# luciddreamer-cvlab/LucidDreamer

Measured on AMD Instinct MI355X. Metric: views/sec fwd+bwd @1080p (1e6 Gaussians), higher is better.
Workload: dtype f32

## Files before the change

luciddreamer_amd/csrc/api.hip:

```cpp
#include "common.h"
#include "lr_src_hash.h"

#include <cstdio>
#include <cstdlib>
#include <cstddef>
#include <cstring>
#include <cmath>
#include <initializer_list>
#include <map>
#include <atomic>
#include <chrono>
#include <mutex>
#include <thread>
#include <string>
#include <vector>

namespace {

thread_local std::string g_last_error;

int fail(int code, const std::string& msg)
{
    g_last_error = msg;
    return code;
}

bool weight_ok(float w) { return w >= 0.f && std::isfinite(w); }

#define LR_HIP_CHECK(expr)                                                                        \
    do {                                                                                          \
        hipError_t e__ = (expr);                                                                  \
        if (e__ != hipSuccess)                                                                    \
            return fail(LR_ERR_HIP, std::string(#expr) + ": " + hipGetErrorString(e__));          \
    } while (0)

#define LR_DEBUG_SYNC(debug, stream, what)                                                        \
    do {                                                                                          \
        if (debug) {                                                                              \
            hipError_t e__ = hipStreamSynchronize(stream);                                        \
            if (e__ == hipSuccess) e__ = hipGetLastError();                                       \
            if (e__ != hipSuccess)                                                                \
                return fail(LR_ERR_HIP, std::string("[HIP ERROR] after ") + what + ": " + hipGetErrorString(e__)); \
        }                                                                                         \
    } while (0)

enum Stage { ST_PREPROCESS = 0, ST_COMPACT, ST_BIN_COUNT, ST_BIN_SCAN, ST_BIN_SCATTER, ST_TILE_SORT, ST_RENDER_FWD,
             ST_GRAD_ZERO, ST_RENDER_BWD, ST_OUT_ZERO, ST_GAUSS_BWD, ST_COUNT };
const char* const kStageNames[ST_COUNT] = { "preprocess", "compact", "bin_count", "bin_scan", "bin_scatter", "tile_sort",
                                            "render_fwd", "grad_zero", "render_bwd", "out_zero", "gauss_bwd" };
struct ProfRec { int stage; hipEvent_t e0, e1; };
bool g_prof_on = false;
std::mutex g_prof_mu;
std::vector<ProfRec> g_prof_recs;
std::vector<hipEvent_t> g_prof_pool;

hipEvent_t prof_event()
{
    {
        std::lock_guard<std::mutex> lock(g_prof_mu);
        if (!g_prof_pool.empty()) { hipEvent_t e = g_prof_pool.back(); g_prof_pool.pop_back(); return e; }
    }
    hipEvent_t e = nullptr;
    (void)hipEventCreate(&e);
    return e;
}
struct ProfScope {
    hipStream_t s; ProfRec r; bool on;
    ProfScope(int stage, hipStream_t s_) : s(s_), on(g_prof_on)
    {
        if (on) { r.stage = stage; r.e0 = prof_event(); r.e1 = prof_event(); (void)hipEventRecord(r.e0, s); }
    }
    ~ProfScope()
    {
        if (on) { (void)hipEventRecord(r.e1, s); std::lock_guard<std::mutex> lock(g_prof_mu); g_prof_recs.push_back(r); }
    }
};

struct BinProf : lr::TileBinTimes {
    ProfRec cur; bool open = false;
    void mark(int boundary, hipStream_t s) override
    {
        if (!g_prof_on) return;
        if (open) { (void)hipEventRecord(cur.e1, s); std::lock_guard<std::mutex> lock(g_prof_mu); g_prof_recs.push_back(cur); open = false; }
        if (boundary < 4) {
            cur.stage = ST_BIN_COUNT + boundary; cur.e0 = prof_event(); cur.e1 = prof_event();
            (void)hipEventRecord(cur.e0, s); open = true;
        }
    }
};

struct TuneTable { int v[lr::TUNE_COUNT]; TuneTable() { for (int& x : v) x = -1; } } g_tune_table;
int* const g_tune = g_tune_table.v;
const char* const kTuneNames[] = { "bwd_red", "blend_quad", "tile_map", "preprocess", "gauss_bwd", "tsort", "walk_own", "hit_mask", "views_in_flight", "strict", "part_scan", "bwd_seg", "fwd_pair", "pcull" };
static_assert(sizeof(kTuneNames) / sizeof(kTuneNames[0]) == lr::TUNE_COUNT, "one name per TuneKey");

std::mutex g_hint_mu;
std::map<std::pair<int, uint32_t>, float> g_vis_frac;
std::map<std::pair<int, uint32_t>, uint32_t> g_inst_hint;
constexpr float kSparseViewFraction = 0.30f;

void view_hint_note(int device, uint32_t P, uint32_t num_compact, uint32_t num_instances)
{
    if (P == 0) return;
    std::lock_guard<std::mutex> lock(g_hint_mu);
    g_vis_frac[std::make_pair(device, P)] = (float)num_compact / (float)P;
    g_inst_hint[std::make_pair(device, P)] = num_instances;
}
long long view_hint_instances(int device, uint32_t P)
{
    std::lock_guard<std::mutex> lock(g_hint_mu);
    auto it = g_inst_hint.find(std::make_pair(device, P));
    return it != g_inst_hint.end() ? (long long)it->second : -1;
}
bool view_hint_sparse(int device, uint32_t P)
{
    std::lock_guard<std::mutex> lock(g_hint_mu);
    auto it = g_vis_frac.find(std::make_pair(device, P));
    return it != g_vis_frac.end() && it->second <= kSparseViewFraction;
}

thread_local bool g_early_request = false;
thread_local long long g_early_ticket = -1;

struct StreamScratch { uint32_t* words = nullptr; size_t n = 0; bool dirty = false; };
std::mutex g_scratch_mu;
std::map<std::pair<int, hipStream_t>, StreamScratch> g_scratch;
StreamScratch* stream_scratch(hipStream_t s, size_t n_words)
{
    int device = 0;
    if (hipGetDevice(&device) != hipSuccess) return nullptr;
    StreamScratch* sc;
    {
        std::lock_guard<std::mutex> lock(g_scratch_mu);
        sc = &g_scratch[std::make_pair(device, s)];
    }
    if (sc->n < n_words) {
        uint32_t* w = nullptr;
        const size_t cap = n_words + n_words / 2 + 64;
        if (hipMalloc(reinterpret_cast<void**>(&w), cap * 4) != hipSuccess) return nullptr;
        if (hipMemsetAsync(w, 0, cap * 4, s) != hipSuccess) return nullptr;
        sc->words = w; sc->n = cap; sc->dirty = false;
    } else if (sc->dirty) {
        if (hipMemsetAsync(sc->words, 0, sc->n * 4, s) != hipSuccess) return nullptr;
        sc->dirty = false;
    }
    return sc;
}

constexpr int kLogSlots = 4096, kLogWords = 12;
constexpr long long kLogTicketBit = 1ll << 40;
struct ForwardLog { uint32_t* host = nullptr; uint32_t* dev = nullptr; std::atomic<long long> next{0}; };
std::mutex g_log_mu;
std::map<int, ForwardLog*> g_logs;
ForwardLog* forward_log(int device)
{
    std::lock_guard<std::mutex> lock(g_log_mu);
    auto it = g_logs.find(device);
    if (it != g_logs.end()) return it->second;
    ForwardLog* L = new ForwardLog();
    const size_t bytes = (size_t)kLogSlots * kLogWords * 4;
    if (hipHostMalloc(reinterpret_cast<void**>(&L->host), bytes, hipHostMallocMapped | hipHostMallocCoherent) != hipSuccess ||
        hipHostGetDevicePointer(reinterpret_cast<void**>(&L->dev), L->host, 0) != hipSuccess) {
        delete L;
        g_logs[device] = nullptr;
        return nullptr;
    }
    std::memset(L->host, 0, bytes);
    g_logs[device] = L;
    return L;
}
thread_local long long g_last_forward_ticket = -1;

thread_local hipEvent_t g_bwd_wait_event = nullptr;
hipEvent_t take_backward_wait_event() { hipEvent_t e = g_bwd_wait_event; g_bwd_wait_event = nullptr; return e; }

thread_local bool g_reset_sticky = false;
// ... 186 lines not shown
    if (P > 0 && (!v.means3D || !v.opacities || !radii)) return fail(LR_ERR_INVALID_ARG, "means3D/opacities/radii are required");
    if (P > 0 && v.shs == nullptr && v.colors_precomp == nullptr)
        return fail(LR_ERR_INVALID_ARG, "For non-RGB, provide precomputed Gaussian colors!");
    if (P > 0 && v.cov3D_precomp == nullptr && (v.scales == nullptr || v.rotations == nullptr))
        return fail(LR_ERR_INVALID_ARG, "provide scales+rotations or cov3D_precomp");
    if (v.shs != nullptr && (D < 0 || D > 3 || (D + 1) * (D + 1) > M))
        return fail(LR_ERR_INVALID_ARG, "SH degree must be 0..3 and (D+1)^2 <= M");
    if (binning_capacity < 0 || binning_capacity > 0xFFFFFFF0ll) return fail(LR_ERR_INVALID_ARG, "bad binning_capacity");

    const ViewParams vp = view_params(v);
    const int num_tiles = vp.gx * vp.gy;

    char* geom = a.geom_alloc(geom_layout(P).total, a.geom_user);
    char* img = a.img_alloc(img_layout(width, height).total, a.img_user);
    if (!geom || !img) return fail(LR_ERR_ALLOC, "geom/img allocator returned NULL");
    const GeomView gv = geom_view(geom, P);
    const ImgView iv = img_view(img, width, height);
    BinView bv = {};

    const size_t n_sum_words = chunk_sum_words(P);
    StreamScratch* scratch = P > 0 ? stream_scratch(s, n_sum_words) : nullptr;
    if (P > 0 && !scratch) return fail(LR_ERR_ALLOC, "could not allocate the per-stream scratch");
    struct DirtyOnError { StreamScratch* sc; bool armed; ~DirtyOnError() { if (sc && armed) sc->dirty = true; } } guard{ scratch, false };
    g_last_forward_ticket = -1;

    long long R_bound = 0;
    int num_rendered = 0;
    bool ranges_written = false;
    long long inst_hint = -1;

    if (P > 0) {
        int device = 0;
        (void)hipGetDevice(&device);
        inst_hint = view_hint_instances(device, (uint32_t)P);
        { ProfScope ps(ST_PREPROCESS, s);
        launch_preprocess(vp, v, a.prefiltered != 0, radii, gv, scratch->words, view_hint_sparse(device, (uint32_t)P), antialiasing, s); }
        guard.armed = true;
        LR_DEBUG_SYNC(debug, s, "preprocess");

        uint32_t* log_slot = nullptr;
        uint32_t log_tag = 0;
#ifdef LR_DIAGNOSTICS
        static const bool no_log = [] { const char* e = getenv("LR_NO_FWD_LOG"); return e && atoi(e) != 0; }();
#else
        constexpr bool no_log = false;
#endif
        if (binning_capacity != 0 && !no_log) {
            if (ForwardLog* L = forward_log(device)) {
                const long long seq = L->next.fetch_add(1);
                log_slot = L->dev + (size_t)(seq % kLogSlots) * kLogWords;
                log_tag = (uint32_t)(seq + 1);
                g_last_forward_ticket = ((long long)device << 41) | kLogTicketBit | (seq & (kLogTicketBit - 1));
            }
        }
        { ProfScope ps(ST_COMPACT, s);
        launch_compact(P, gv, reinterpret_cast<const uint4*>(scratch->words), (uint32_t)binning_capacity, log_slot, log_tag,
                       { iv.bin_total, (uint32_t)part_plan(num_tiles).bins }, reset_sticky, s); }
        LR_DEBUG_SYNC(debug, s, "compact");

        if (binning_capacity == 0) {
            GeomHeader h;
            LR_HIP_CHECK(hipMemcpyAsync(&h, gv.header, offsetof(GeomHeader, n_seg), hipMemcpyDeviceToHost, s));
            LR_HIP_CHECK(hipStreamSynchronize(s));
            view_hint_note(device, (uint32_t)P, h.num_compact, h.num_instances);
            R_bound = h.num_instances;
            if (h.num_rendered > 0x7FFFFFFFu)
                return fail(LR_ERR_INVALID_ARG, "num_rendered exceeds INT_MAX: use async mode (binning_capacity > 0) and read the count with lr_check");
            num_rendered = (int)h.num_rendered;
        } else {
            R_bound = binning_capacity;
            num_rendered = LR_NUM_RENDERED_ON_DEVICE;
            if (early_header) {
                g_early_ticket = g_last_forward_ticket >= 0 ? g_last_forward_ticket : lr_header_post(geom, a.stream);
                if (g_early_ticket < 0) return (int)g_early_ticket;
            }
        }

        char* bin = a.binning_alloc(bin_layout(R_bound).total, a.binning_user);
        if (!bin) return fail(LR_ERR_ALLOC, "binning allocator returned NULL");
        bv = bin_view(bin, R_bound);
        if (R_bound > 0) {
            BinProf bp;
            const int rc = launch_tile_binning(vp, bits_for((uint32_t)(R_bound - 1)), gv, iv, bv, radii, R_bound, &bp,
                                               { scratch->words, (uint32_t)n_sum_words }, s);
            if (rc == -2) return fail(LR_ERR_INVALID_ARG, "image / instance count too large: tile and slot bits exceed the 64-bit sort word");
            if (rc != 0) return fail(LR_ERR_HIP, "could not reserve LDS for the binning kernels");
            ranges_written = true;
            guard.armed = false;
            LR_DEBUG_SYNC(debug, s, "tile binning");
        }
    } else {
        (void)a.binning_alloc(bin_layout(0).total, a.binning_user);
    }
    if (!ranges_written) LR_HIP_CHECK(hipMemsetAsync(iv.ranges, 0, (size_t)num_tiles * sizeof(uint2), s));

    { ProfScope ps(ST_RENDER_FWD, s);
    launch_render_fwd(vp, gv, iv, bv, v.background, a.out_color, a.out_depth, inst_hint, s); }
    LR_DEBUG_SYNC(debug, s, "render");
    LR_HIP_CHECK(hipGetLastError());

    if (binning_capacity == 0 && a.prefiltered && P > 0) {
        uint32_t trap = 0;
        LR_HIP_CHECK(hipMemcpyAsync(&trap, &gv.header->prefilter_trap, 4, hipMemcpyDeviceToHost, s));
        LR_HIP_CHECK(hipStreamSynchronize(s));
        if (trap) return fail(LR_ERR_PREFILTERED, "Point is filtered although prefiltered is set. This shouldn't happen!");
    }
    return num_rendered;
}

static const char* const kUncoveredMsg =
    "lr_backward: R / binning_capacity are smaller than the forward's -- the blend backward's launch did not reach every list "
    "segment and the gradients of this view are incomplete (pass the value lr_forward returned / was given)";

static void zero_fill_write_rows(const lr::GradOut& out, float* dL_dsh_rest, int P, int M, bool raw, hipStream_t s)
{
    using namespace lr;
    const unsigned int accumulate_mask = out.accumulate_mask;
    float* const dL_dmean2D_abs = out.mean2D_abs;
    const unsigned long long Pn = (unsigned long long)P;
    const unsigned long long nsh = raw ? 3 * Pn : (unsigned long long)M * 3 * Pn;
    const unsigned long long nf[ACC_ROWS] = { 3 * Pn, 4 * Pn, Pn, 3 * Pn, 3 * Pn, 6 * Pn, nsh, 3 * Pn, 4 * Pn };
    float* zp[11]; unsigned long long zn[11]; int zc = 0;
    const bool no_fill = (accumulate_mask & LR_ACC_NO_ZERO_FILL) != 0u;
    for (int k = 0; k < ACC_ROWS; k++)
        if (out.row[k] != nullptr && !((accumulate_mask >> k) & 1u) && (!no_fill || k == ACC_MEAN2D)) { zp[zc] = out.row[k]; zn[zc] = nf[k]; zc++; }
    if (!no_fill && raw && dL_dsh_rest != nullptr && M > 1 && !((accumulate_mask >> ACC_SH) & 1u) && zc < 9) {
        zp[zc] = dL_dsh_rest; zn[zc] = (unsigned long long)(M - 1) * 3 * Pn; zc++;
    }
    const bool abs_own = dL_dmean2D_abs != nullptr && zc >= 9;
    if (dL_dmean2D_abs != nullptr && !abs_own) { zp[zc] = dL_dmean2D_abs; zn[zc] = 3 * Pn; zc++; }
    if (zc > 0) {
        ProfScope ps(ST_OUT_ZERO, s);
        launch_zero_outputs(zp, zn, zc, s);
        if (abs_own) { float* one = dL_dmean2D_abs; const unsigned long long n = 3 * Pn; launch_zero_outputs(&one, &n, 1, s); }
    }
}

static int backward_core(const lr_backward_args& a, hipEvent_t wait_before_accumulate, float* acc16, float* stat_accum = nullptr,
                         bool stat_abs = false)
{
    using namespace lr;
    const bool antialiasing = g_antialiasing.load(std::memory_order_relaxed) != 0;
    const lr_view& v = a.view;
    const int P = v.P, M = v.M, width = v.width, height = v.height, debug = a.debug;
    const bool raw = v.raw != 0;
    char* const geom_buffer = a.geom_buffer; char* const binning_buffer = a.binning_buffer; char* const image_buffer = a.image_buffer;
    const unsigned int accumulate_mask = a.accumulate_mask;
    const bool depth = a.dL_depths != nullptr && a.depth_image != nullptr;
    hipStream_t s = reinterpret_cast<hipStream_t>(a.stream);
    if (P <= 0) return 0;
    if (!geom_buffer || !binning_buffer || !image_buffer) return fail(LR_ERR_INVALID_ARG, "scratch buffers are required");
    if (!a.dL_dpix || !a.dL_dmean2D || !a.dL_dopacity || !a.dL_dmean3D)
        return fail(LR_ERR_INVALID_ARG, "gradient outputs dL_dmean2D/dL_dopacity/dL_dmean3D are required");
    if (v.colors_precomp != nullptr && !a.dL_dcolor) return fail(LR_ERR_INVALID_ARG, "dL_dcolor is required with colors_precomp");
    if (v.cov3D_precomp != nullptr && !a.dL_dcov3D) return fail(LR_ERR_INVALID_ARG, "dL_dcov3D is required with cov3D_precomp");
    if (v.scales != nullptr && (!a.dL_dscale || !a.dL_drot)) return fail(LR_ERR_INVALID_ARG, "dL_dscale/dL_drot are required with scales");
    if (v.shs != nullptr && a.dL_dsh == nullptr) return fail(LR_ERR_INVALID_ARG, "dL_dsh is required when shs is given");
    if (const int rc = all_aligned16("backward", "gradient outputs", { a.dL_dmean2D, a.dL_dconic, a.dL_dopacity, a.dL_dcolor, a.dL_dmean3D,
                                     a.dL_dcov3D, a.dL_dsh, a.dL_dscale, a.dL_drot, a.dL_dsh_rest, a.dL_dmean2D_abs })) return rc;

    const GeomView gv = geom_view(geom_buffer, P);
    const ImgView iv = img_view(image_buffer, width, height);
    const BinView bv = bin_view_list(binning_buffer);
    const long long seg_bound = (a.binning_capacity > 0 || a.R > 0)
                                    ? bin_seg_capacity(a.binning_capacity > 0 ? a.binning_capacity : (long long)a.R) : -1;

    const ViewParams vp = view_params(v, true, a.dL_dsh_rest);
// ... 1594 lines not shown
int lr_step_abort(void)
{
    int device = 0;
    LR_HIP_CHECK(hipGetDevice(&device));
    std::lock_guard<std::mutex> lock(g_step_mu);
    StepAcc& g = g_step[device];
    g.active = false; g.armed = false;
    return 0;
}

long long lr_forward_ticket(void) { return g_last_forward_ticket; }
void lr_backward_wait_event(void* event) { g_bwd_wait_event = reinterpret_cast<hipEvent_t>(event); }

static int forward_log_poll(long long ticket, int block, unsigned int* out8)
{
    const int device = (int)(ticket >> 41);
    const long long seq = ticket & (kLogTicketBit - 1);
    ForwardLog* L;
    {
        std::lock_guard<std::mutex> lock(g_log_mu);
        auto it = g_logs.find(device);
        L = it == g_logs.end() ? nullptr : it->second;
    }
    if (!L) return fail(LR_ERR_INVALID_ARG, "lr_header_poll: unknown forward-log ticket");
    const uint32_t want = (uint32_t)(seq + 1);
    volatile uint32_t* slot = L->host + (size_t)(seq % kLogSlots) * kLogWords;
    const auto t0 = std::chrono::steady_clock::now();
    for (int spin = 0;; spin++) {
        const uint32_t tag = __atomic_load_n(const_cast<uint32_t*>(slot), __ATOMIC_ACQUIRE);
        if (tag == want) break;
        if (tag != 0 && (int32_t)(tag - want) > 0)
            return fail(LR_ERR_INVALID_ARG, "lr_header_poll: the forward log has wrapped past this ticket (more than 4096 forwards were outstanding)");
        if (!block) return 0;
        if ((spin & 63) == 63) {
            std::this_thread::yield();
            if (std::chrono::steady_clock::now() - t0 > std::chrono::seconds(30))
                return fail(LR_ERR_HIP, "lr_header_poll: the forward of this ticket did not reach its scan within 30 s");
        }
    }
    if (out8) for (int i = 0; i < 8; i++) out8[i] = slot[1 + i];
    view_hint_note(device, slot[1 + LR_HDR_WORD(P)], slot[1 + LR_HDR_WORD(num_compact)], slot[1 + LR_HDR_WORD(num_instances)]);
    return 1;
}

int lr_header_poll(long long ticket, int block, unsigned int* out8)
{
    if (ticket >= 0 && (ticket & kLogTicketBit)) return forward_log_poll(ticket, block, out8);
    HeaderTicket h;
    {
        std::lock_guard<std::mutex> lock(g_hdr_mu);
        if (ticket < 0 || (size_t)ticket >= g_hdr_tickets.size() || !g_hdr_tickets[(size_t)ticket].busy)
            return fail(LR_ERR_INVALID_ARG, "lr_header_poll: unknown ticket");
        h = g_hdr_tickets[(size_t)ticket];
    }
    hipError_t q = block ? hipEventSynchronize(h.ev) : hipEventQuery(h.ev);
    if (q == hipErrorNotReady) return 0;
    if (q != hipSuccess) {
        header_ticket_release(ticket);
        return fail(LR_ERR_HIP, std::string("lr_header_poll: ") + hipGetErrorString(q));
    }
    if (out8) for (int i = 0; i < 8; i++) out8[i] = h.host[i];
    view_hint_note(h.device, h.host[LR_HDR_WORD(P)], h.host[LR_HDR_WORD(num_compact)], h.host[LR_HDR_WORD(num_instances)]);
    header_ticket_release(ticket);
    return 1;
}

void lr_request_early_header(void) { g_early_request = true; g_early_ticket = -1; }
long long lr_take_early_ticket(void) { const long long t = g_early_ticket; g_early_ticket = -1; g_early_request = false; return t; }

int lr_set_antialiasing(int on) { return g_antialiasing.exchange(on != 0 ? 1 : 0); }
int lr_get_antialiasing(void) { return g_antialiasing.load(); }

int lr_tune_set(const char* name, int value)
{
    if (!name) return fail(LR_ERR_INVALID_ARG, "lr_tune_set: NULL name");
    for (int i = 0; i < lr::TUNE_COUNT; i++)
        if (std::strcmp(name, kTuneNames[i]) == 0) {
#ifndef LR_DIAGNOSTICS
            if ((i == lr::TUNE_PART_SCAN && value >= 0) || (i == lr::TUNE_BWD_RED && (value == 0 || value == 2 || value == 3)) ||
                (i == lr::TUNE_FWD_PAIR && value == 1))
                return fail(LR_ERR_INVALID_ARG, std::string("lr_tune_set: ") + name + " = " + std::to_string(value) +
                            " selects a retired kernel (diagnostics build only: python -m luciddreamer_amd.build --diagnostics)");
#endif
            g_tune[i] = value;
            return 0;
        }
    return fail(LR_ERR_INVALID_ARG, std::string("lr_tune_set: unknown knob ") + name);
}

int lr_last_launch_shapes(int* forward_shape, int* backward_shape)
{
    if (forward_shape) *forward_shape = lr::last_fwd_shape();
    if (backward_shape) *backward_shape = lr::last_bwd_shape();
    return 0;
}

int lr_last_forward_channels(int* channels)
{
    if (channels) *channels = lr::last_fwd_channels();
    return 0;
}

int lr_profile_enable(int on)
{
    std::lock_guard<std::mutex> lock(g_prof_mu);
    for (auto& r : g_prof_recs) { g_prof_pool.push_back(r.e0); g_prof_pool.push_back(r.e1); }
    g_prof_recs.clear();
    g_prof_on = on != 0;
    return ST_COUNT;
}

const char* lr_profile_stage_name(int stage) { return (stage >= 0 && stage < ST_COUNT) ? kStageNames[stage] : ""; }

int lr_profile_read(double* ms_per_stage, long long* calls_per_stage, int n_stages)
{
    if (!ms_per_stage || !calls_per_stage || n_stages < ST_COUNT) return fail(LR_ERR_INVALID_ARG, "need ST_COUNT slots");
    for (int i = 0; i < n_stages; i++) { ms_per_stage[i] = 0.0; calls_per_stage[i] = 0; }
    std::lock_guard<std::mutex> lock(g_prof_mu);
    for (auto& r : g_prof_recs) {
        LR_HIP_CHECK(hipEventSynchronize(r.e1));
        float ms = 0.f;
        LR_HIP_CHECK(hipEventElapsedTime(&ms, r.e0, r.e1));
        ms_per_stage[r.stage] += ms;
        calls_per_stage[r.stage] += 1;
    }
    return ST_COUNT;
}

size_t lr_dist2_workspace_bytes(int P) { return lr::dist2_workspace_bytes(P); }

int lr_dist2_workspace_layout(int P, size_t offsets[4])
{
    if (P < 0) return fail(LR_ERR_INVALID_ARG, "P must be >= 0");
    if (!offsets) return fail(LR_ERR_INVALID_ARG, "NULL argument");
    lr::dist2_workspace_layout(P, offsets);
    return 0;
}

int lr_dist2(int P, const float* points, float* out, char* workspace, void* stream_)
{
    hipStream_t s = reinterpret_cast<hipStream_t>(stream_);
    if (P < 0) return fail(LR_ERR_INVALID_ARG, "P must be >= 0");
    if (P == 0) return 0;
    if (!points || !out || !workspace) return fail(LR_ERR_INVALID_ARG, "NULL argument");
    lr::launch_dist2(P, points, out, workspace, s);
    LR_HIP_CHECK(hipGetLastError());
    return 0;
}

}
```

luciddreamer_amd/csrc/common.h:

```cpp
#pragma once
#include <hip/hip_runtime.h>
#include <stdint.h>
#include <stddef.h>
#include "screen_cull.h"
#include "gauss_project.h"
#include "../../include/lucid_raster.h"

namespace lr {

constexpr int TILE_PIX = TILE_X * TILE_Y;
constexpr int WAVE = 64;

struct __attribute__((aligned(16))) GaussRec {
    float x, y, ca, cb;
    float cc, opacity, r, g;
    float b, depth, qmax, pad1;
};
static_assert(sizeof(GaussRec) == 48, "GaussRec must be 48 bytes");

struct __attribute__((aligned(16))) GradRec {
    float dmx, dmy, dca, dcb;
    float dcc, dop, dr, dg;
    float db, pad0, pad1, pad2;
};
// ... 201 lines not shown
{
#pragma clang fp contract(off)
    const float t = Cp * dy;
    return t * dy;
}
__device__ __forceinline__ float gauss_power1(float Ap, float Bd, float Cdd, float dx)
{
    return __builtin_fmaf(__builtin_fmaf(Ap, dx, Bd), dx, Cdd);
}
template <bool STRICT>
__device__ __forceinline__ void gauss_row(float qB, float qC, float dy, float& r0, float& r1)
{
    if (STRICT) { r0 = dy; r1 = 0.f; }
    else { r0 = gauss_bd(qB, dy); r1 = gauss_cdd(qC, dy); }
}
__device__ __forceinline__ float gauss_power_strict(float ca, float cb, float cc, float dx, float dy)
{
#pragma clang fp contract(off)
    return -0.5f * (ca * dx * dx + cc * dy * dy) - cb * dx * dy;
}
__device__ __forceinline__ float strict_expf(float x)
{
#pragma clang fp contract(off)
    const float c = 0x1.715476p+0f, cc = 0x1.4ae0bep-26f;
    const float ph = x * c;
    const float pl = __builtin_fmaf(x, cc, __builtin_fmaf(x, c, -ph));
    const float e = __builtin_rintf(ph);
    const float a = (ph - e) + pl;
    return __builtin_ldexpf(__builtin_amdgcn_exp2f(a), (int)e);
}
template <bool STRICT>
__device__ __forceinline__ float gauss_weight(float qA, float qB, float qC, float r0, float r1, float dx, float& power)
{
    if (STRICT) {
        power = gauss_power_strict(qA, qB, qC, dx, r0);
        return strict_expf(power);
    }
    power = gauss_power1(qA, r0, r1, dx);
    return __builtin_amdgcn_exp2f(power);
}

constexpr float LOG2E = 1.4426950408889634f;
constexpr float LN2 = 0.6931471805599453f;
__device__ __forceinline__ float gauss_exp2(float power2) { return __builtin_amdgcn_exp2f(power2); }

struct ViewParams {
    const float* view;
    const float* proj;
    const float* campos;
    float tan_fovx, tan_fovy, focal_x, focal_y, scale_modifier;
    int W, H, gx, gy, P, D, M;
    int hit_origin_limit;
    int raw;
    const float* sh_rest;
    const float* opacity_raw;
    float* dL_dsh_rest;
    ScreenCull cull;
    int pcull;
};

__device__ __forceinline__ float act_scale(float s) { return expf(s); }
__device__ __forceinline__ float act_opacity(float o) { return 1.0f / (1.0f + expf(-o)); }
__device__ __forceinline__ float act_quat_inv_norm(float r, float x, float y, float z)
{
    return 1.0f / fmaxf(sqrtf(r * r + x * x + y * y + z * z), 1e-12f);
}

struct WordSpan { uint32_t* words; uint32_t n; };
void launch_preprocess(const ViewParams& vp, const lr_view& v, bool prefiltered, int* radii, const GeomView& g,
                       uint32_t* chunk_sums, bool sparse_view_hint, bool antialiasing, hipStream_t s);
inline size_t chunk_sum_words(int P) { return 4 * (((size_t)(P > 0 ? P : 1) + SCAN_TILE - 1) / SCAN_TILE) + 1; }
void launch_mark_visible(int P, const float* means3D, const float* view, const float* proj, uint8_t* present,
                         hipStream_t s);

inline int radix_sort_passes(int end_bit) { return (end_bit + RADIX_BITS - 1) / RADIX_BITS; }
void radix_sort_pairs(uint32_t* key_a, uint32_t* key_b, uint32_t* val_a, uint32_t* val_b, bool vals_iota,
                      const uint32_t* n_dev, long long n_bound, int end_bit, uint32_t* hist,
                      uint32_t** keys_out, uint32_t** vals_out, hipStream_t s);

void launch_compact(int P, const GeomView& g, const uint4* block_sums, uint32_t capacity, uint32_t* log_slot, uint32_t log_tag,
                    WordSpan zero, bool reset_sticky, hipStream_t s);
struct TileBinTimes { virtual void mark(int boundary, hipStream_t s) = 0; virtual ~TileBinTimes() {} };
int launch_tile_binning(const ViewParams& vp, int slot_bits, const GeomView& g, const ImgView& im, const BinView& b,
                        const int* radii, long long bin_bound_hint, TileBinTimes* t, WordSpan clear, hipStream_t s);

enum TuneKey { TUNE_BWD_RED = 0, TUNE_BLEND_QUAD, TUNE_TILE_MAP, TUNE_PREPROCESS, TUNE_GAUSS_BWD, TUNE_TSORT, TUNE_WALK_OWN, TUNE_HIT_MASK, TUNE_VIEWS_IN_FLIGHT, TUNE_STRICT, TUNE_PART_SCAN, TUNE_BWD_SEG, TUNE_FWD_PAIR, TUNE_PCULL, TUNE_COUNT };
int tune_get(int key);

enum { BLEND_HALF = 0, BLEND_QUAD = 1, BLEND_TILE = 2 };
int blend_shape(int num_tiles, long long inst_bound = -1);
struct ViewsInFlight { explicit ViewsInFlight(int n); ~ViewsInFlight(); int prev; };
int views_in_flight();
void note_fwd_shape(int shape);
int last_fwd_shape();
int last_bwd_shape();
enum { FWD_CHANNEL_COLOR = 1, FWD_CHANNEL_DEPTH = 2 };
void note_fwd_channels(int channels);
int last_fwd_channels();
enum { TILE_MAP_BANDS = 0, TILE_MAP_PLAIN = 1 };
int blend_tile_map(int num_tiles);
__device__ __forceinline__ int blend_tile(int map, int num_tiles)
{
    int t = (int)blockIdx.x;
    if (map == TILE_MAP_BANDS) {
        const int per = (num_tiles + 7) >> 3;
        t = (int)(blockIdx.x & 7) * per + (int)(blockIdx.x >> 3);
    }
    return t < num_tiles ? t : -1;
}
void launch_render_fwd(const ViewParams& vp, const GeomView& g, const ImgView& im, const BinView& b, const float* bg,
                       float* out_color, float* out_depth, long long inst_hint, hipStream_t s);
void launch_render_alpha(const float* final_T, long long n, float* alpha, hipStream_t s);
void launch_render_median(int W, int H, int P, const GeomView& g, const ImgView& im, const char* bin_base, float* out_depth,
                          int* out_ids, hipStream_t s);
void launch_median_bwd(int W, int H, int P, const GeomView& g, const int* radii, const int* ids, const float* dL_dmedian,
                       const float* view, float* dL_dmean3D, bool accumulate, hipStream_t s);
void launch_render_distort(int W, int H, int P, const GeomView& g, const ImgView& im, const char* bin_base, float c0, float c1,
                           float c2, float* out_distortion, float* out_moments, hipStream_t s);
void launch_distort_bwd(int W, int H, int P, const GeomView& g, const ImgView& im, char* bin_base, const float* dL_ddistortion,
                        const float* distortion, const float* moments, float c0, float c1, float c2, hipStream_t s);
void launch_gauss_normals(int P, bool raw, const float* means3D, const float* scales, const float* rotations, const float* view,
                          const int* radii, float* out_gauss_normals, hipStream_t s);
void launch_render_normals(int W, int H, int P, const GeomView& g, const ImgView& im, const char* bin_base,
                           const float* gauss_normals, float* out_normals, hipStream_t s);
void launch_normals_bwd(int W, int H, int P, const GeomView& g, const ImgView& im, char* bin_base, const float* dL_dnormals,
                        const float* normals, const float* gauss_normals, hipStream_t s);
void launch_normal_rot_bwd(int P, bool raw, const float* rotations, const float* view, const int* radii, const GeomView& g,
                           const float* gauss_normals, const float* dL_dgauss_normal, float* dL_drot, hipStream_t s);
int features_chunk();
size_t features_workspace_bytes(long long slots);
void launch_render_features(int W, int H, int P, const GeomView& g, const ImgView& im, const char* bin_base, const float* features,
                            int C, float* out_features, hipStream_t s);
void launch_features_bwd(int W, int H, int P, const GeomView& g, const ImgView& im, char* bin_base, const float* dL_dout_features,
                         const float* out_features, const float* features, int C, char* workspace, size_t workspace_bytes,
                         bool accumulate, float* dL_dfeatures, hipStream_t s);
void launch_render_geom(int W, int H, int P, const GeomView& g, const ImgView& im, const char* bin_base, const float* gauss_normals,
                        float c0, float c1, float c2, float* out_distortion, float* out_moments, float* out_normals, hipStream_t s);
void launch_geom_bwd(int W, int H, int P, const GeomView& g, const ImgView& im, char* bin_base, const float* dL_ddistortion,
                     float dist_scalar, const float* distortion, const float* moments, float c0, float c1, float c2,
                     const float* dL_dnormals, const float* normals, const float* gauss_normals, hipStream_t s);
struct ViewGrads {
    const float* color;
    const float* depth;
    const float* alpha;
    const float* depth_img;
};
void launch_render_bwd(const ViewParams& vp, const GeomView& g, const ImgView& im, const BinView& b, const float* bg,
                       const ViewGrads& up, bool absgrad, long long seg_bound, hipStream_t s);
__device__ __forceinline__ void adam_one(float gi, float& mi, float& vi, float& pi, float w1, float beta2, float w2,
                                         float bc2_sqrt, float eps, float step_size)
{
    mi = __builtin_fmaf(w1, gi - mi, mi);
    vi = vi * beta2;
    vi = __builtin_fmaf(w2 * gi, gi, vi);
    const float denom = sqrtf(vi) / bc2_sqrt + eps;
    pi = __builtin_fmaf(-step_size, mi / denom, pi);
}
enum { ACC_MEAN2D = 0, ACC_CONIC = 1, ACC_OPACITY = 2, ACC_COLOR = 3, ACC_MEAN3D = 4, ACC_COV3D = 5, ACC_SH = 6,
       ACC_SCALE = 7, ACC_ROT = 8, ACC_ROWS = 9 };
struct GradOut {
    float* row[ACC_ROWS];
    float* mean2D_abs;
    uint32_t accumulate_mask;
    float* acc16;
    float* stat_accum;
    bool stat_abs;
};
void launch_gauss_bwd(const ViewParams& vp, const lr_view& v, const GeomView& g, const BinView& b, const GradOut& out,
                      bool depth, bool antialiasing, hipStream_t s);
// ... 183 lines not shown
```

luciddreamer_amd/csrc/tilebin.hip:

```cpp
#include <mutex>
#include "common.h"

namespace lr {

namespace {

__device__ __forceinline__ uint64_t lanemask_lt()
{
    const uint32_t lane = threadIdx.x & 63;
    return (lane == 0) ? 0ull : (~0ull >> (64 - lane));
}

__device__ __forceinline__ uint32_t block_reduce_sum(uint32_t v, uint32_t* s_tmp)
{
#pragma unroll
    for (int off = 32; off > 0; off >>= 1) v += __shfl_down(v, off);
    if ((threadIdx.x & 63) == 0) s_tmp[threadIdx.x >> 6] = v;
    lds_barrier();
    uint32_t t = 0;
    for (int i = 0; i < (int)(blockDim.x >> 6); i++) t += s_tmp[i];
    lds_barrier();
    return t;
}

// ... 445 lines not shown
                                                uint32_t* s_wave, uint32_t* s_bad_p, int tid, Sync sync)
{
    const int lane = tid & 63, w = tid >> 6;
    unsigned long long item[PER];
    unsigned long long kmin = ~0ull, kmax = 0ull;
#pragma unroll
    for (int k = 0; k < PER; k++) {
        const uint32_t i = (uint32_t)tid + (uint32_t)k * THREADS;
        item[k] = i < n ? src[i] : ~0ull;
        if (i < n) { const unsigned long long key = item[k] >> slot_bits; kmin = key < kmin ? key : kmin; kmax = key > kmax ? key : kmax; }
    }
#pragma unroll
    for (int k = 0; k < PER; k++) s_cnt[tid + k * THREADS] = 0u;
    if (tid == 0) *s_bad_p = 0u;
#pragma unroll
    for (int off = 32; off > 0; off >>= 1) {
        const unsigned long long a = __shfl_xor(kmin, off), b = __shfl_xor(kmax, off);
        kmin = a < kmin ? a : kmin; kmax = b > kmax ? b : kmax;
    }
    if (lane == 0) { s_red[2 * w] = kmin; s_red[2 * w + 1] = kmax; }
    sync();
#pragma unroll
    for (int i = 0; i < THREADS / 64; i++) { kmin = s_red[2 * i] < kmin ? s_red[2 * i] : kmin; kmax = s_red[2 * i + 1] > kmax ? s_red[2 * i + 1] : kmax; }
    uint32_t nb = 1;
    while (nb < n) nb <<= 1;
    const double scale = (double)nb / ((double)(kmax - kmin) + 1.0);
    uint32_t bucket[PER];
#pragma unroll
    for (int k = 0; k < PER; k++) {
        const uint32_t i = (uint32_t)tid + (uint32_t)k * THREADS;
        uint32_t bk = (uint32_t)((double)((item[k] >> slot_bits) - kmin) * scale);
        bucket[k] = bk < nb ? bk : nb - 1;
        if (i < n) atomicAdd(&s_cnt[bucket[k]], 1u);
    }
    sync();
    uint32_t c[PER], sum = 0;
#pragma unroll
    for (int k = 0; k < PER; k++) { c[k] = s_cnt[tid * PER + k]; sum += c[k]; if (c[k] > 32u) *s_bad_p = 1u; }
    uint32_t inc = sum;
#pragma unroll
    for (int off = 1; off < 64; off <<= 1) {
        const uint32_t t = __shfl_up(inc, off);
        if (lane >= off) inc += t;
    }
    if (lane == 63) s_wave[w] = inc;
    sync();
    uint32_t run = inc - sum;
    for (int j = 0; j < w; j++) run += s_wave[j];
    const uint32_t my_first = run;
#pragma unroll
    for (int k = 0; k < PER; k++) { s_cnt[tid * PER + k] = run; run += c[k]; }
    sync();
#pragma unroll
    for (int k = 0; k < PER; k++) {
        const uint32_t i = (uint32_t)tid + (uint32_t)k * THREADS;
        if (i < n) s_out[atomicAdd(&s_cnt[bucket[k]], 1u)] = item[k];
    }
    sync();
    if (*s_bad_p) {
        bitonic_sort(s_out, n, (uint32_t)tid, (uint32_t)THREADS, sync);
    } else {
        uint32_t lo = my_first;
#pragma unroll
        for (int k = 0; k < PER; k++) {
            const uint32_t hi = lo + c[k];
            for (uint32_t i = lo + 1; i < hi; i++) {
                const unsigned long long x = s_out[i];
                uint32_t j = i;
                while (j > lo && s_out[j - 1] > x) { s_out[j] = s_out[j - 1]; j--; }
                s_out[j] = x;
            }
            lo = hi;
        }
        sync();
    }
}

__global__ void __launch_bounds__(256)
k_tile_sort_small(int bins, int groups4, int sub_shift, int slot_bits, int num_tiles, int bucket_b, int rank_max, const uint32_t* __restrict__ bin_start,
                  const uint32_t* __restrict__ bin_total, const unsigned long long* __restrict__ words,
                  uint32_t* __restrict__ point_list, uint2* __restrict__ ranges, const uint32_t* __restrict__ inst_gid,
                  uint32_t* __restrict__ list_gid)
{
    __shared__ __attribute__((aligned(16))) unsigned long long s_a[4 * TSORT_LDS];
    __shared__ uint32_t s_cnt[TSORT_GROUP_LDS];
    __shared__ unsigned long long s_red[8];
    __shared__ uint32_t s_wave[4];
    __shared__ uint32_t s_bad[4];
    const int w = threadIdx.x >> 6, l = threadIdx.x & 63;
    if ((int)blockIdx.x < groups4) {
        const int bin = (int)blockIdx.x * 4 + w;
        const uint32_t n = bin < bins ? bin_total[bin] : 0u;
        const uint32_t start = bin < bins ? bin_start[bin] : 0u;
        if (n == 0 || n > (uint32_t)TSORT_LDS) return;
        unsigned long long* a = s_a + w * TSORT_LDS;
        auto wsync = [] { __builtin_amdgcn_fence(__ATOMIC_RELEASE, "wavefront"); __builtin_amdgcn_wave_barrier();
                          __builtin_amdgcn_fence(__ATOMIC_ACQUIRE, "wavefront"); };
        if (n <= (uint32_t)rank_max) {
            const uint32_t un = (uint32_t)__builtin_amdgcn_readfirstlane((int)n), ustart = (uint32_t)__builtin_amdgcn_readfirstlane((int)start);
            const unsigned long long* src = words + ustart;
            if (un <= 64u) rank_sort_wave<1>(src, un, a, ustart, bin, sub_shift, slot_bits, num_tiles, (uint32_t)l, point_list, ranges, inst_gid, list_gid, wsync);
            else if (un <= 128u) rank_sort_wave<2>(src, un, a, ustart, bin, sub_shift, slot_bits, num_tiles, (uint32_t)l, point_list, ranges, inst_gid, list_gid, wsync);
            else rank_sort_wave<4>(src, un, a, ustart, bin, sub_shift, slot_bits, num_tiles, (uint32_t)l, point_list, ranges, inst_gid, list_gid, wsync);
            return;
        }
        if (bucket_b == 2 && n > 64) {
            bucket_sort_bin<64, TSORT_LDS / 64>(words + start, n, slot_bits, a, s_cnt + w * TSORT_LDS, s_red + 2 * w, s_wave + w,
                                                &s_bad[w], l, wsync);
            write_sorted(a, n, start, bin, sub_shift, slot_bits, num_tiles, (uint32_t)l, 64u, point_list, ranges, inst_gid, list_gid);
            return;
        }
        for (uint32_t i = l; i < n; i += 64) a[i] = words[start + i];
        wsync();
        if (n > 1) bitonic_sort(a, n, (uint32_t)l, 64u, wsync);
        write_sorted(a, n, start, bin, sub_shift, slot_bits, num_tiles, (uint32_t)l, 64u, point_list, ranges, inst_gid, list_gid);
        return;
    }
    const int first = (int)blockIdx.x - groups4, stride = (int)gridDim.x - groups4;
    for (int bin = first; bin < bins; bin += stride) {
        const uint32_t n = bin_total[bin];
        if (n <= (uint32_t)TSORT_LDS || n > (uint32_t)TSORT_GROUP_LDS) continue;
        const uint32_t start = bin_start[bin];
        lds_barrier();
        if (bucket_b) {
            bucket_sort_bin<256, TSORT_GROUP_LDS / 256>(words + start, n, slot_bits, s_a, s_cnt, s_red, s_wave, &s_bad[0],
                                                        (int)threadIdx.x, [] { lds_barrier(); });
        } else {
            for (uint32_t i = threadIdx.x; i < n; i += 256) s_a[i] = words[start + i];
            lds_barrier();
            bitonic_sort(s_a, n, threadIdx.x, 256u, [] { lds_barrier(); });
        }
        write_sorted(s_a, n, start, bin, sub_shift, slot_bits, num_tiles, threadIdx.x, 256u, point_list, ranges, inst_gid, list_gid);
    }
}

__global__ void __launch_bounds__(TSORT_THREADS)
k_tile_sort_large(int sub_shift, int slot_bits, int num_tiles, uint32_t lds_entries, const uint32_t* __restrict__ bin_start,
                  const uint32_t* __restrict__ bin_total, unsigned long long* __restrict__ words,
                  uint32_t* __restrict__ point_list, uint2* __restrict__ ranges, const uint32_t* __restrict__ big_queue,
                  const uint32_t* __restrict__ inst_gid, uint32_t* __restrict__ list_gid)
{
    constexpr int PER = TSORT_MID_LDS / TSORT_THREADS;
    extern __shared__ unsigned long long s_out[];
    __shared__ uint32_t s_cnt[TSORT_MID_LDS];
    __shared__ unsigned long long s_red[2 * (TSORT_THREADS / 64)];
    __shared__ uint32_t s_wave[TSORT_THREADS / 64];
    __shared__ uint32_t s_bad;
    const int tid = threadIdx.x;
    const uint32_t count = big_queue[0];
    for (uint32_t qi = blockIdx.x; qi < count; qi += gridDim.x) {
    const int bin = (int)big_queue[1 + qi];
    const uint32_t n = bin_total[bin];
    const uint32_t start = bin_start[bin];
    lds_barrier();
    if (n > (uint32_t)TSORT_MID_LDS) {
        if (n <= lds_entries) {
            for (uint32_t i = tid; i < n; i += TSORT_THREADS) s_out[i] = words[start + i];
            lds_barrier();
            bitonic_sort(s_out, n, (uint32_t)tid, (uint32_t)TSORT_THREADS, [] { lds_barrier(); });
            write_sorted(s_out, n, start, bin, sub_shift, slot_bits, num_tiles, (uint32_t)tid, (uint32_t)TSORT_THREADS, point_list, ranges, inst_gid, list_gid);
        } else {
            unsigned long long* a = words + start;
            bitonic_sort(a, n, (uint32_t)tid, (uint32_t)TSORT_THREADS, [] { __threadfence(); lds_barrier(); });
            write_sorted(a, n, start, bin, sub_shift, slot_bits, num_tiles, (uint32_t)tid, (uint32_t)TSORT_THREADS, point_list, ranges, inst_gid, list_gid);
        }
        continue;
    }
    bucket_sort_bin<TSORT_THREADS, PER>(words + start, n, slot_bits, s_out, s_cnt, s_red, s_wave, &s_bad, tid, [] { lds_barrier(); });
    write_sorted(s_out, n, start, bin, sub_shift, slot_bits, num_tiles, (uint32_t)tid, (uint32_t)TSORT_THREADS, point_list, ranges, inst_gid, list_gid);
    }
}

}

PartPlan part_plan(int num_tiles)
{
    PartPlan p;
    p.sub_shift = 0;
    while (((num_tiles - 1) >> p.sub_shift) + 1 > PART_BINS_MAX) p.sub_shift++;
    p.bins = num_tiles > 0 ? ((num_tiles - 1) >> p.sub_shift) + 1 : 1;
    return p;
}

void launch_compact(int P, const GeomView& g, const uint4* block_sums, uint32_t capacity, uint32_t* log_slot, uint32_t log_tag,
                    WordSpan zero, bool reset_sticky, hipStream_t s)
{
    const int nb = (P + SCAN_TILE - 1) / SCAN_TILE;
    hipLaunchKernelGGL(k_compact_write, dim3(nb), dim3(SCAN_THREADS), 0, s, P, g.tiles_touched, block_sums, g.vis_list,
                       g.offsets, g.header, capacity, log_slot, log_tag, zero.words, zero.n, reset_sticky ? 1 : 0);
}

int launch_tile_binning(const ViewParams& vp, int slot_bits, const GeomView& g, const ImgView& im, const BinView& b,
                        const int* radii, long long bin_bound_hint, TileBinTimes* t, WordSpan clear, hipStream_t s)
{
    const int P = vp.P, gx = vp.gx, gy = vp.gy;
    {
        static std::mutex mu;
        static bool attr_done[64] = {};
        int device = 0;
        if (hipGetDevice(&device) != hipSuccess) return -1;
        std::lock_guard<std::mutex> lock(mu);
        if (device < 0 || device >= 64 || !attr_done[device]) {
            if (hipFuncSetAttribute(reinterpret_cast<const void*>(k_part<0>), hipFuncAttributeMaxDynamicSharedMemorySize,
                                    (PART_BINS_MAX + PART_BINS_MAX / 16 + 1) * 4) != hipSuccess ||
                hipFuncSetAttribute(reinterpret_cast<const void*>(k_part<1>), hipFuncAttributeMaxDynamicSharedMemorySize,
                                    (PART_BINS_MAX + PART_BINS_MAX / 16 + 1) * 4) != hipSuccess ||
                hipFuncSetAttribute(reinterpret_cast<const void*>(k_tile_sort_large), hipFuncAttributeMaxDynamicSharedMemorySize,
                                    TSORT_BIG_LDS * 8) != hipSuccess)
                return -1;
            if (device >= 0 && device < 64) attr_done[device] = true;
        }
    }
    const int num_tiles = gx * gy;
    const PartPlan pp = part_plan(num_tiles);
    if (pp.sub_shift + 31 + slot_bits > 64) return -2;
    long long nb = ((long long)P + PART_MIN_GAUSS - 1) / PART_MIN_GAUSS;
    if (nb < 1) nb = 1;
    if (nb > PART_BLOCKS_MAX) nb = PART_BLOCKS_MAX;
    const size_t lds = ((size_t)pp.bins + pp.bins / 16 + 1) * 4;
    const int own_max = tune_get(TUNE_WALK_OWN) >= 0 ? tune_get(TUNE_WALK_OWN) : 12;
#ifdef LR_DIAGNOSTICS
    const int reserve = tune_get(TUNE_PART_SCAN) == 1 ? 0 : 1;
#else
    constexpr int reserve = 1;
#endif
    if (t) t->mark(0, s);
#define LR_PART_ARGS gx, gy, pp.bins, pp.sub_shift, slot_bits, own_max, g.vis_list, g.offsets, g.hitrec, g.rec, radii, g.header,     \
                     im.part_hist, im.bin_total, im.bin_start, im.ranges, im.big_queue, b.inst_gid, b.words
    hipLaunchKernelGGL(k_part<0>, dim3((unsigned)nb), dim3(PART_THREADS), lds, s, LR_PART_ARGS, clear.words, clear.n, reserve);
#ifdef LR_DIAGNOSTICS
    if (!reserve) {
        if (t) t->mark(1, s);
        hipLaunchKernelGGL(k_part_scan1, dim3((pp.bins + SCAN1_BINS - 1) / SCAN1_BINS), dim3(SCAN1_BINS * SCAN1_GROUPS), 0, s, pp.bins,
                           g.header, im.part_hist, im.bin_total);
    }
#endif
    if (t) t->mark(2, s);
    hipLaunchKernelGGL(k_part<1>, dim3((unsigned)nb), dim3(PART_THREADS), lds, s, LR_PART_ARGS, nullptr, 0u, reserve);
#undef LR_PART_ARGS
    if (t) t->mark(3, s);
    const int groups4 = (pp.bins + 3) / 4;
    const int part_b = pp.bins < TSORT_CLASS_BLOCKS ? pp.bins : TSORT_CLASS_BLOCKS;
    const int tsort = tune_get(TUNE_TSORT);
    const int bucket_b = (tsort >= 0 && tsort <= 2) ? tsort : 2;
    const int rank_max = tsort < 0 ? TSORT_RANK_DEFAULT : (tsort == 3 ? TSORT_LDS : (tsort == 4 ? 128 : 0));
    hipLaunchKernelGGL(k_tile_sort_small, dim3(groups4 + part_b), dim3(256), 0, s, pp.bins, groups4, pp.sub_shift, slot_bits,
                       num_tiles, bucket_b, rank_max, im.bin_start, im.bin_total, b.words, b.point_list, im.ranges, b.inst_gid, b.list_gid);
    const long long avg_bin = bin_bound_hint / (long long)pp.bins;
    const bool huge = avg_bin > (long long)TSORT_MID_LDS;
    const uint32_t lds_entries = huge ? (uint32_t)TSORT_BIG_LDS : (uint32_t)TSORT_MID_LDS;
    const int large_cap = huge ? TSORT_BIG_BLOCKS : (avg_bin <= (long long)TSORT_LDS ? TSORT_LARGE_BLOCKS / 12 : TSORT_LARGE_BLOCKS);
    const int large_blocks = pp.bins < large_cap ? pp.bins : large_cap;
    hipLaunchKernelGGL(k_tile_sort_large, dim3(large_blocks), dim3(TSORT_THREADS), (size_t)lds_entries * 8, s, pp.sub_shift,
                       slot_bits, num_tiles, lds_entries, im.bin_start, im.bin_total, b.words, b.point_list, im.ranges, im.big_queue,
                       b.inst_gid, b.list_gid);
    if (t) t->mark(4, s);
    return hipGetLastError() == hipSuccess ? 0 : -1;
}

}
```

Baseline: 6351.

## Fuse per-bin small and large tile sorts into one kernel in async mode

Adds k_tile_sort_resid, which runs the small-bin sort body and then drains the big-bin queue itself. Bins too large for LDS are sorted in place in global memory with a block-local bitonic sort plus global merge steps. It replaces the separate k_tile_sort_large launch when binning runs async and the average bin is small, aiming to cut one launch and its tail. The cost is that oversized bins get a slower single-workgroup sort with many global syncs, and the small-bin blocks also wait on queue work.

```diff
diff --git a/luciddreamer_amd/csrc/api.hip b/luciddreamer_amd/csrc/api.hip
--- a/luciddreamer_amd/csrc/api.hip
+++ b/luciddreamer_amd/csrc/api.hip
@@ -91,7 +91,7 @@
 
 struct TuneTable { int v[lr::TUNE_COUNT]; TuneTable() { for (int& x : v) x = -1; } } g_tune_table;
 int* const g_tune = g_tune_table.v;
-const char* const kTuneNames[] = { "bwd_red", "blend_quad", "tile_map", "preprocess", "gauss_bwd", "tsort", "walk_own", "hit_mask", "views_in_flight", "strict", "part_scan", "bwd_seg", "fwd_pair", "pcull" };
+const char* const kTuneNames[] = { "bwd_red", "blend_quad", "tile_map", "preprocess", "gauss_bwd", "tsort", "walk_own", "hit_mask", "views_in_flight", "strict", "part_scan", "bwd_seg", "fwd_pair", "pcull", "bin_fuse" };
 static_assert(sizeof(kTuneNames) / sizeof(kTuneNames[0]) == lr::TUNE_COUNT, "one name per TuneKey");
 
 std::mutex g_hint_mu;
@@ -444,7 +444,8 @@
         if (R_bound > 0) {
             BinProf bp;
             const int rc = launch_tile_binning(vp, bits_for((uint32_t)(R_bound - 1)), gv, iv, bv, radii, R_bound, &bp,
-                                               { scratch->words, (uint32_t)n_sum_words }, s);
+                                               { scratch->words, (uint32_t)n_sum_words },
+                                               binning_capacity != 0 && tune_get(TUNE_BIN_FUSE) != 0, s);
             if (rc == -2) return fail(LR_ERR_INVALID_ARG, "image / instance count too large: tile and slot bits exceed the 64-bit sort word");
             if (rc != 0) return fail(LR_ERR_HIP, "could not reserve LDS for the binning kernels");
             ranges_written = true;
@@ -2205,6 +2206,8 @@
                 return fail(LR_ERR_INVALID_ARG, std::string("lr_tune_set: ") + name + " = " + std::to_string(value) +
                             " selects a retired kernel (diagnostics build only: python -m luciddreamer_amd.build --diagnostics)");
 #endif
+            if (i == lr::TUNE_BIN_FUSE && (value < -1 || value > 1))
+                return fail(LR_ERR_INVALID_ARG, "lr_tune_set: bin_fuse is -1 (the library's rule: one per-bin sort launch in async mode), 0 (two) or 1");
             g_tune[i] = value;
             return 0;
         }
diff --git a/luciddreamer_amd/csrc/common.h b/luciddreamer_amd/csrc/common.h
--- a/luciddreamer_amd/csrc/common.h
+++ b/luciddreamer_amd/csrc/common.h
@@ -307,9 +307,9 @@
                     WordSpan zero, bool reset_sticky, hipStream_t s);
 struct TileBinTimes { virtual void mark(int boundary, hipStream_t s) = 0; virtual ~TileBinTimes() {} };
 int launch_tile_binning(const ViewParams& vp, int slot_bits, const GeomView& g, const ImgView& im, const BinView& b,
-                        const int* radii, long long bin_bound_hint, TileBinTimes* t, WordSpan clear, hipStream_t s);
-
-enum TuneKey { TUNE_BWD_RED = 0, TUNE_BLEND_QUAD, TUNE_TILE_MAP, TUNE_PREPROCESS, TUNE_GAUSS_BWD, TUNE_TSORT, TUNE_WALK_OWN, TUNE_HIT_MASK, TUNE_VIEWS_IN_FLIGHT, TUNE_STRICT, TUNE_PART_SCAN, TUNE_BWD_SEG, TUNE_FWD_PAIR, TUNE_PCULL, TUNE_COUNT };
+                        const int* radii, long long bin_bound_hint, TileBinTimes* t, WordSpan clear, bool one_sort, hipStream_t s);
+
+enum TuneKey { TUNE_BWD_RED = 0, TUNE_BLEND_QUAD, TUNE_TILE_MAP, TUNE_PREPROCESS, TUNE_GAUSS_BWD, TUNE_TSORT, TUNE_WALK_OWN, TUNE_HIT_MASK, TUNE_VIEWS_IN_FLIGHT, TUNE_STRICT, TUNE_PART_SCAN, TUNE_BWD_SEG, TUNE_FWD_PAIR, TUNE_PCULL, TUNE_BIN_FUSE, TUNE_COUNT };
 int tune_get(int key);
 
 enum { BLEND_HALF = 0, BLEND_QUAD = 1, BLEND_TILE = 2 };
diff --git a/luciddreamer_amd/csrc/tile_sort_small_body.h b/luciddreamer_amd/csrc/tile_sort_small_body.h
--- /dev/null
+++ b/luciddreamer_amd/csrc/tile_sort_small_body.h
@@ -0,0 +1,50 @@
+    __shared__ __attribute__((aligned(16))) unsigned long long s_a[4 * TSORT_LDS];
+    __shared__ uint32_t s_cnt[TSORT_GROUP_LDS];
+    __shared__ unsigned long long s_red[8];
+    __shared__ uint32_t s_wave[4];
+    __shared__ uint32_t s_bad[4];
+    const int w = threadIdx.x >> 6, l = threadIdx.x & 63;
+    if ((int)blockIdx.x < groups4) {
+        const int bin = (int)blockIdx.x * 4 + w;
+        const uint32_t n = bin < bins ? bin_total[bin] : 0u;
+        const uint32_t start = bin < bins ? bin_start[bin] : 0u;
+        if (n == 0 || n > (uint32_t)TSORT_LDS) return;
+        unsigned long long* a = s_a + w * TSORT_LDS;
+        auto wsync = [] { __builtin_amdgcn_fence(__ATOMIC_RELEASE, "wavefront"); __builtin_amdgcn_wave_barrier();
+                          __builtin_amdgcn_fence(__ATOMIC_ACQUIRE, "wavefront"); };
+        if (n <= (uint32_t)rank_max) {
+            const uint32_t un = (uint32_t)__builtin_amdgcn_readfirstlane((int)n), ustart = (uint32_t)__builtin_amdgcn_readfirstlane((int)start);
+            const unsigned long long* src = words + ustart;
+            if (un <= 64u) rank_sort_wave<1>(src, un, a, ustart, bin, sub_shift, slot_bits, num_tiles, (uint32_t)l, point_list, ranges, inst_gid, list_gid, wsync);
+            else if (un <= 128u) rank_sort_wave<2>(src, un, a, ustart, bin, sub_shift, slot_bits, num_tiles, (uint32_t)l, point_list, ranges, inst_gid, list_gid, wsync);
+            else rank_sort_wave<4>(src, un, a, ustart, bin, sub_shift, slot_bits, num_tiles, (uint32_t)l, point_list, ranges, inst_gid, list_gid, wsync);
+            return;
+        }
+        if (bucket_b == 2 && n > 64) {
+            bucket_sort_bin<64, TSORT_LDS / 64>(words + start, n, slot_bits, a, s_cnt + w * TSORT_LDS, s_red + 2 * w, s_wave + w,
+                                                &s_bad[w], l, wsync);
+            write_sorted(a, n, start, bin, sub_shift, slot_bits, num_tiles, (uint32_t)l, 64u, point_list, ranges, inst_gid, list_gid);
+            return;
+        }
+        for (uint32_t i = l; i < n; i += 64) a[i] = words[start + i];
+        wsync();
+        if (n > 1) bitonic_sort(a, n, (uint32_t)l, 64u, wsync);
+        write_sorted(a, n, start, bin, sub_shift, slot_bits, num_tiles, (uint32_t)l, 64u, point_list, ranges, inst_gid, list_gid);
+        return;
+    }
+    const int first = (int)blockIdx.x - groups4, stride = (int)gridDim.x - groups4;
+    for (int bin = first; bin < bins; bin += stride) {
+        const uint32_t n = bin_total[bin];
+        if (n <= (uint32_t)TSORT_LDS || n > (uint32_t)TSORT_GROUP_LDS) continue;
+        const uint32_t start = bin_start[bin];
+        lds_barrier();
+        if (bucket_b) {
+            bucket_sort_bin<256, TSORT_GROUP_LDS / 256>(words + start, n, slot_bits, s_a, s_cnt, s_red, s_wave, &s_bad[0],
+                                                        (int)threadIdx.x, [] { lds_barrier(); });
+        } else {
+            for (uint32_t i = threadIdx.x; i < n; i += 256) s_a[i] = words[start + i];
+            lds_barrier();
+            bitonic_sort(s_a, n, threadIdx.x, 256u, [] { lds_barrier(); });
+        }
+        write_sorted(s_a, n, start, bin, sub_shift, slot_bits, num_tiles, threadIdx.x, 256u, point_list, ranges, inst_gid, list_gid);
+    }
diff --git a/luciddreamer_amd/csrc/tilebin.hip b/luciddreamer_amd/csrc/tilebin.hip
--- a/luciddreamer_amd/csrc/tilebin.hip
+++ b/luciddreamer_amd/csrc/tilebin.hip
@@ -551,55 +551,84 @@
                   uint32_t* __restrict__ point_list, uint2* __restrict__ ranges, const uint32_t* __restrict__ inst_gid,
                   uint32_t* __restrict__ list_gid)
 {
-    __shared__ __attribute__((aligned(16))) unsigned long long s_a[4 * TSORT_LDS];
-    __shared__ uint32_t s_cnt[TSORT_GROUP_LDS];
-    __shared__ unsigned long long s_red[8];
-    __shared__ uint32_t s_wave[4];
-    __shared__ uint32_t s_bad[4];
-    const int w = threadIdx.x >> 6, l = threadIdx.x & 63;
-    if ((int)blockIdx.x < groups4) {
-        const int bin = (int)blockIdx.x * 4 + w;
-        const uint32_t n = bin < bins ? bin_total[bin] : 0u;
-        const uint32_t start = bin < bins ? bin_start[bin] : 0u;
-        if (n == 0 || n > (uint32_t)TSORT_LDS) return;
-        unsigned long long* a = s_a + w * TSORT_LDS;
-        auto wsync = [] { __builtin_amdgcn_fence(__ATOMIC_RELEASE, "wavefront"); __builtin_amdgcn_wave_barrier();
-                          __builtin_amdgcn_fence(__ATOMIC_ACQUIRE, "wavefront"); };
-        if (n <= (uint32_t)rank_max) {
-            const uint32_t un = (uint32_t)__builtin_amdgcn_readfirstlane((int)n), ustart = (uint32_t)__builtin_amdgcn_readfirstlane((int)start);
-            const unsigned long long* src = words + ustart;
-            if (un <= 64u) rank_sort_wave<1>(src, un, a, ustart, bin, sub_shift, slot_bits, num_tiles, (uint32_t)l, point_list, ranges, inst_gid, list_gid, wsync);
-            else if (un <= 128u) rank_sort_wave<2>(src, un, a, ustart, bin, sub_shift, slot_bits, num_tiles, (uint32_t)l, point_list, ranges, inst_gid, list_gid, wsync);
-            else rank_sort_wave<4>(src, un, a, ustart, bin, sub_shift, slot_bits, num_tiles, (uint32_t)l, point_list, ranges, inst_gid, list_gid, wsync);
-            return;
-        }
-        if (bucket_b == 2 && n > 64) {
-            bucket_sort_bin<64, TSORT_LDS / 64>(words + start, n, slot_bits, a, s_cnt + w * TSORT_LDS, s_red + 2 * w, s_wave + w,
-                                                &s_bad[w], l, wsync);
-            write_sorted(a, n, start, bin, sub_shift, slot_bits, num_tiles, (uint32_t)l, 64u, point_list, ranges, inst_gid, list_gid);
-            return;
-        }
-        for (uint32_t i = l; i < n; i += 64) a[i] = words[start + i];
-        wsync();
-        if (n > 1) bitonic_sort(a, n, (uint32_t)l, 64u, wsync);
-        write_sorted(a, n, start, bin, sub_shift, slot_bits, num_tiles, (uint32_t)l, 64u, point_list, ranges, inst_gid, list_gid);
-        return;
-    }
-    const int first = (int)blockIdx.x - groups4, stride = (int)gridDim.x - groups4;
-    for (int bin = first; bin < bins; bin += stride) {
+#include "tile_sort_small_body.h"
+}
+
+__device__ __forceinline__ void bitonic_step(unsigned long long* a, uint32_t n, uint32_t half, uint32_t lk, uint32_t lj, uint32_t tid,
+                                             uint32_t nthreads)
+{
+    const uint32_t k = 1u << lk, j = 1u << lj;
+    const bool flip = (lj == lk - 1);
+    for (uint32_t c = tid; c < half; c += nthreads) {
+        const uint32_t hi = c >> lj, lo = c & (j - 1u);
+        uint32_t i, l;
+        if (flip) { i = (hi << lk) + lo; l = i ^ (k - 1u); }
+        else { i = (hi << (lj + 1u)) + lo; l = i + j; }
+        if (l < n) {
+            const unsigned long long x = a[i], y = a[l];
+            if (x > y) { a[i] = y; a[l] = x; }
+        }
+    }
+}
+
+constexpr uint32_t RESID_LB = 10;
+static_assert((1u << RESID_LB) == (uint32_t)TSORT_GROUP_LDS, "a block is what the workgroup's LDS holds");
+
+__device__ __forceinline__ void sort_bin_in_place(unsigned long long* a, uint32_t n, unsigned long long* s_a, uint32_t tid)
+{
+    constexpr uint32_t B = 1u << RESID_LB;
+    auto gsync = [] { __threadfence(); lds_barrier(); };
+    for (uint32_t off = 0; off < n; off += B) {
+        const uint32_t m = n - off < B ? n - off : B;
+        for (uint32_t i = tid; i < m; i += 256) s_a[i] = a[off + i];
+        lds_barrier();
+        for (uint32_t lk = 1; lk <= RESID_LB; lk++)
+            for (uint32_t lj = lk; lj-- > 0;) {
+                bitonic_step(s_a, m, B >> 1, lk, lj, tid, 256u);
+                lds_barrier();
+            }
+        for (uint32_t i = tid; i < m; i += 256) a[off + i] = s_a[i];
+        lds_barrier();
+    }
+    gsync();
+    uint32_t lm = 0;
+    while ((1u << lm) < n) lm++;
+    const uint32_t half = 1u << (lm - 1);
+    for (uint32_t lk = RESID_LB + 1; lk <= lm; lk++) {
+        for (uint32_t lj = lk; lj-- > RESID_LB;) {
+            bitonic_step(a, n, half, lk, lj, tid, 256u);
+            gsync();
+        }
+        for (uint32_t off = 0; off < n; off += B) {
+            const uint32_t m = n - off < B ? n - off : B;
+            for (uint32_t i = tid; i < m; i += 256) s_a[i] = a[off + i];
+            lds_barrier();
+            for (uint32_t lj = RESID_LB; lj-- > 0;) {
+                bitonic_step(s_a, m, B >> 1, lk, lj, tid, 256u);
+                lds_barrier();
+            }
+            for (uint32_t i = tid; i < m; i += 256) a[off + i] = s_a[i];
+            lds_barrier();
+        }
+        gsync();
+    }
+}
+
+__global__ void __launch_bounds__(256) __attribute__((amdgpu_waves_per_eu(8, 8)))
+k_tile_sort_resid(int bins, int groups4, int sub_shift, int slot_bits, int num_tiles, int bucket_b, int rank_max, const uint32_t* __restrict__ bin_start,
+                  const uint32_t* __restrict__ bin_total, unsigned long long* words,
+                  uint32_t* __restrict__ point_list, uint2* __restrict__ ranges, const uint32_t* __restrict__ inst_gid,
+                  uint32_t* __restrict__ list_gid, const uint32_t* __restrict__ big_queue)
+{
+#include "tile_sort_small_body.h"
+    const uint32_t count = big_queue[0];
+    for (uint32_t qi = (uint32_t)first; qi < count; qi += (uint32_t)stride) {
+        const int bin = (int)big_queue[1 + qi];
         const uint32_t n = bin_total[bin];
-        if (n <= (uint32_t)TSORT_LDS || n > (uint32_t)TSORT_GROUP_LDS) continue;
         const uint32_t start = bin_start[bin];
         lds_barrier();
-        if (bucket_b) {
-            bucket_sort_bin<256, TSORT_GROUP_LDS / 256>(words + start, n, slot_bits, s_a, s_cnt, s_red, s_wave, &s_bad[0],
-                                                        (int)threadIdx.x, [] { lds_barrier(); });
-        } else {
-            for (uint32_t i = threadIdx.x; i < n; i += 256) s_a[i] = words[start + i];
-            lds_barrier();
-            bitonic_sort(s_a, n, threadIdx.x, 256u, [] { lds_barrier(); });
-        }
-        write_sorted(s_a, n, start, bin, sub_shift, slot_bits, num_tiles, threadIdx.x, 256u, point_list, ranges, inst_gid, list_gid);
+        sort_bin_in_place(words + start, n, s_a, threadIdx.x);
+        write_sorted(words + start, n, start, bin, sub_shift, slot_bits, num_tiles, threadIdx.x, 256u, point_list, ranges, inst_gid, list_gid);
     }
 }
 
@@ -660,7 +689,7 @@
 }
 
 int launch_tile_binning(const ViewParams& vp, int slot_bits, const GeomView& g, const ImgView& im, const BinView& b,
-                        const int* radii, long long bin_bound_hint, TileBinTimes* t, WordSpan clear, hipStream_t s)
+                        const int* radii, long long bin_bound_hint, TileBinTimes* t, WordSpan clear, bool one_sort, hipStream_t s)
 {
     const int P = vp.P, gx = vp.gx, gy = vp.gy;
     {
@@ -713,9 +742,16 @@
     const int tsort = tune_get(TUNE_TSORT);
     const int bucket_b = (tsort >= 0 && tsort <= 2) ? tsort : 2;
     const int rank_max = tsort < 0 ? TSORT_RANK_DEFAULT : (tsort == 3 ? TSORT_LDS : (tsort == 4 ? 128 : 0));
+    const long long avg_bin = bin_bound_hint / (long long)pp.bins;
+    if (one_sort && avg_bin <= (long long)TSORT_LDS) {
+        hipLaunchKernelGGL(k_tile_sort_resid, dim3(groups4 + part_b), dim3(256), 0, s, pp.bins, groups4, pp.sub_shift, slot_bits,
+                           num_tiles, bucket_b, rank_max, im.bin_start, im.bin_total, b.words, b.point_list, im.ranges, b.inst_gid, b.list_gid,
+                           im.big_queue);
+        if (t) t->mark(4, s);
+        return hipGetLastError() == hipSuccess ? 0 : -1;
+    }
     hipLaunchKernelGGL(k_tile_sort_small, dim3(groups4 + part_b), dim3(256), 0, s, pp.bins, groups4, pp.sub_shift, slot_bits,
                        num_tiles, bucket_b, rank_max, im.bin_start, im.bin_total, b.words, b.point_list, im.ranges, b.inst_gid, b.list_gid);
-    const long long avg_bin = bin_bound_hint / (long long)pp.bins;
     const bool huge = avg_bin > (long long)TSORT_MID_LDS;
     const uint32_t lds_entries = huge ? (uint32_t)TSORT_BIG_LDS : (uint32_t)TSORT_MID_LDS;
     const int large_cap = huge ? TSORT_BIG_BLOCKS : (avg_bin <= (long long)TSORT_LDS ? TSORT_LARGE_BLOCKS / 12 : TSORT_LARGE_BLOCKS);
```

Result: faster. 6463, median of 6 (+1.8%).
